# mengcaopku/DCNet

Measured on AMD Instinct MI355X. Metric: clips/sec (T=8, 416x416, bs8) fwd+bwd, higher is better.
Workload: dtype f32; 1 GPU; T=8 416x416 bs8/GPU L=20 fp32, 64 img/GPU/step as pairs, fwd+5 losses+bwd+RMSprop; arith=f16x2-split MFMA, fp32 accumulate, parallelism=dp1, ranks_seen=1, reducer=none, step=hipGraph replay (fwd+losses+bwd+RMSprop), sampler=mt

## Files before the change

dcnet_amd/csrc/coattn.hip:

```cpp
#include "igemm.h"
#include "prof.h"

int tn_gemm_batched(const float* A, int lda, long long a_bs, const float* B, int ldb, long long b_bs,
                    float* C, int ldc, long long c_bs, const float* row_scale,
                    int M, int m_ld, int N, int K, int batch, int accumulate, hipStream_t stream,
                    const unsigned* amax_a = nullptr, const unsigned* amax_b = nullptr);

namespace {

constexpr int EXP_ROWS = 32;

typedef _Float16 f16x4c_t __attribute__((ext_vector_type(4)));
constexpr float E_SPLIT_SCALE = 8192.f;
template <bool SPLIT>
__global__ __launch_bounds__(256) void exp_sums_kernel(float* __restrict__ E, int hw, int ldE, float t,
                                                       float* __restrict__ rsum, float* __restrict__ colpart) {
  __shared__ float red[4][EXP_ROWS];
  const int b = blockIdx.y, rb = blockIdx.x;
  const int i0 = rb * EXP_ROWS;
  float* e = E + ((size_t)b * hw + i0) * ldE;
  float racc[EXP_ROWS];
#pragma unroll
  for (int r = 0; r < EXP_ROWS; ++r) racc[r] = 0.f;
  const int nrow = min(EXP_ROWS, hw - i0);
  for (int j = threadIdx.x * 4; j < ldE; j += 1024) {
    f32x4 v[EXP_ROWS];
#pragma unroll
    for (int r = 0; r < EXP_ROWS; ++r)
      v[r] = r < nrow ? *reinterpret_cast<const f32x4*>(e + (size_t)r * ldE + j) : f32x4{0.f, 0.f, 0.f, 0.f};
    f32x4 cs = {0.f, 0.f, 0.f, 0.f};
#pragma unroll
    for (int r = 0; r < EXP_ROWS; ++r) {
      if (r < nrow) {
        f32x4 o;
#pragma unroll
        for (int k = 0; k < 4; ++k) o[k] = (j + k < hw) ? expf(t * v[r][k] - t) : 0.f;
        if constexpr (SPLIT) {
          const f32x4 ts = o * E_SPLIT_SCALE;
          const f16x4c_t h = {(_Float16)ts[0], (_Float16)ts[1], (_Float16)ts[2], (_Float16)ts[3]};
          const f16x4c_t l = {(_Float16)(ts[0] - (float)h[0]), (_Float16)(ts[1] - (float)h[1]), (_Float16)(ts[2] - (float)h[2]),
                              (_Float16)(ts[3] - (float)h[3])};
          unsigned char* run = reinterpret_cast<unsigned char*>(e + (size_t)r * ldE + (j & ~7)) + (j & 4) * 2;
          *reinterpret_cast<f16x4c_t*>(run) = h;
          *reinterpret_cast<f16x4c_t*>(run + 16) = l;
        } else {
          *reinterpret_cast<f32x4*>(e + (size_t)r * ldE + j) = o;
        }
        cs += o; racc[r] += (o[0] + o[1]) + (o[2] + o[3]);
      }
    }
    *reinterpret_cast<f32x4*>(colpart + ((size_t)rb * gridDim.y + b) * ldE + j) = cs;
  }
  const int lane = threadIdx.x & 63, wave = threadIdx.x >> 6;
#pragma unroll
  for (int r = 0; r < EXP_ROWS; ++r) {
    const float s = wave_sum(racc[r]);
    if (lane == 0) red[wave][r] = s;
  }
  __syncthreads();
  if (threadIdx.x < EXP_ROWS && i0 + threadIdx.x < hw)
    rsum[(size_t)b * hw + i0 + threadIdx.x] = 1.f / (red[0][threadIdx.x] + red[1][threadIdx.x] + red[2][threadIdx.x] + red[3][threadIdx.x]);
}

__global__ __launch_bounds__(256) void colsum_inv_kernel(const float* __restrict__ colpart, int nrb, int b, int hw, int ldE,
                                                         float* __restrict__ cinv) {
  const int j = blockIdx.x * 256 + threadIdx.x, bb = blockIdx.y;
  if (j >= hw) return;
  float s = 0.f;
  for (int rb = 0; rb < nrb; ++rb) s += colpart[((size_t)rb * b + bb) * ldE + j];
  cinv[(size_t)bb * hw + j] = 1.f / s;
}

enum { AM_ONE = 0, AM_DO1, AM_DO2, AM_DO1S, AM_DO2S, AM_DA, AM_DP1, AM_DP2, AM_SLOTS };
__global__ __launch_bounds__(256) void amax_init_kernel(unsigned* __restrict__ w) {
  for (int i = threadIdx.x; i < AM_SLOTS * DCN_AMAX_WORDS; i += 256) w[i] = i < DCN_AMAX_WORDS ? 0x3F800000u : 0u;
}

__global__ __launch_bounds__(256) void rowdot_scale_kernel(const float* __restrict__ d, int ldd, int64_t bsd,
                                                           const float* __restrict__ o, int ldo, int64_t bso, int hw,
                                                           const float* __restrict__ inv, int64_t rows, int c,
                                                           float* __restrict__ delta, float* __restrict__ ds,
                                                           unsigned* __restrict__ amax_d, unsigned* __restrict__ amax_ds) {
  __shared__ float red[4];
  const int lane = threadIdx.x & 63;
  const int64_t row = (int64_t)blockIdx.x * 4 + (threadIdx.x >> 6);
  float vmax = 0.f, s = 0.f;
  if (row < rows) {
    const int64_t bb = row / hw, i = row - bb * hw;
    s = inv[row];
    float acc = 0.f;
    for (int k = lane * 4; k < c; k += 256) {
      const f32x4 dv = *reinterpret_cast<const f32x4*>(d + bb * bsd + i * ldd + k);
      const f32x4 ov = *reinterpret_cast<const f32x4*>(o + bb * bso + i * ldo + k);
      acc += dv[0] * ov[0] + dv[1] * ov[1] + dv[2] * ov[2] + dv[3] * ov[3];
      *reinterpret_cast<f32x4*>(ds + row * c + k) = dv * s;
      vmax = fmaxf(fmaxf(vmax, fmaxf(fabsf(dv[0]), fabsf(dv[1]))), fmaxf(fabsf(dv[2]), fabsf(dv[3])));
    }
    acc = wave_sum(acc);
    if (lane == 0) delta[row] = acc;
  }
  const float vs = wave_max(vmax * s);
  amax_update_block(amax_d, vmax, red);
  __syncthreads();
  amax_update_block(amax_ds, vs, red);
// ... 24 lines not shown
      const f16x4c_t h = *reinterpret_cast<const f16x4c_t*>(run), l = *reinterpret_cast<const f16x4c_t*>(run + 16);
#pragma unroll
      for (int k = 0; k < 4; ++k) e[k] = ((float)h[k] + (float)l[k]) * (1.f / E_SPLIT_SCALE);
    } else {
      e = *reinterpret_cast<const f32x4*>(E + row * ldE + j);
    }
    const f32x4 p1 = *reinterpret_cast<const f32x4*>(dP1 + row * ldE + j);
    const f32x4 p2 = *reinterpret_cast<const f32x4*>(dP2 + row * ldE + j);
    const float ri = rinv[row], di = d1[row];
    f32x4 o;
#pragma unroll
    for (int k = 0; k < 4; ++k) {
      float v = 0.f;
      if (j + k < hw) v = t * e[k] * ((p1[k] - di) * ri + (p2[k] - d2[bb * hw + j + k]) * cinv[bb * hw + j + k]);
      o[k] = v;
    }
    if constexpr (OSPLIT) {
      const f32x4 ts = o * s_out;
      const f16x4c_t h = {(_Float16)ts[0], (_Float16)ts[1], (_Float16)ts[2], (_Float16)ts[3]};
      const f16x4c_t l = {(_Float16)(ts[0] - (float)h[0]), (_Float16)(ts[1] - (float)h[1]), (_Float16)(ts[2] - (float)h[2]),
                          (_Float16)(ts[3] - (float)h[3])};
      unsigned char* run = reinterpret_cast<unsigned char*>(dP1 + row * ldE + (j & ~7)) + (j & 4) * 2;
      *reinterpret_cast<f16x4c_t*>(run) = h;
      *reinterpret_cast<f16x4c_t*>(run + 16) = l;
    } else {
      *reinterpret_cast<f32x4*>(dP1 + row * ldE + j) = o;
      vmax = fmaxf(fmaxf(vmax, fmaxf(fabsf(o[0]), fabsf(o[1]))), fmaxf(fabsf(o[2]), fabsf(o[3])));
    }
  }
  if constexpr (!OSPLIT) amax_update_block(amax_da, vmax, red);
}

__global__ __launch_bounds__(64) void da_bound_kernel(const unsigned* __restrict__ a1, const unsigned* __restrict__ a2, float t,
                                                      unsigned* __restrict__ out) {
  const float b = 2.f * t * (__uint_as_float(amax_read(a1)) + __uint_as_float(amax_read(a2)));
  out[threadIdx.x & (DCN_AMAX_WORDS - 1)] = __float_as_uint(b);
}

inline int ld_pad(int hw) { return (hw + 31) / 32 * 32; }

void gemm_params(IgemmParams& p, const float* A, int lda, long long a_bs, const float* B, int ldb, long long b_bs,
                 float* C, int ldc, long long c_bs, int M, int N, int K, int batch) {
  p = IgemmParams{};
  p.osy = p.osx = p.isy = p.isx = 1; p.dense_out = 1;
  p.in = A; p.ldi = lda; p.in_bs = a_bs; p.wt = B; p.ldw = ldb; p.wt_bs = b_bs; p.out = C; p.ldo = ldc; p.out_bs = c_bs;
  p.ldr = ldc;
  p.N = 1; p.Hi = 1; p.Wi = M; p.Ho = 1; p.Wo = M; p.Hs = 1; p.Ws = M; p.M = M;
  p.Ci = K; p.Co = N; p.ntaps = 1; p.batch = batch;
}

}

static bool on_gemm3(int b, int hw, int c) { return c % 32 == 0 && gemm3_applicable(hw, c, hw, b) && gemm3_applicable(hw, hw, c, b); }

extern "C" int64_t dcn_coattn_fwd_ws(int b, int hw, int c) {
  (void)c;
  return (int64_t)cdiv(hw, EXP_ROWS) * b * ld_pad(hw) + AM_SLOTS * DCN_AMAX_WORDS;
}
extern "C" int64_t dcn_coattn_e_size(int b, int hw) { return (int64_t)b * hw * ld_pad(hw); }
extern "C" int64_t dcn_coattn_saved_size(int b, int hw, int c) {
  return dcn_coattn_e_size(b, hw) + (on_gemm3(b, hw, c) ? (int64_t)2 * b * hw * c : 0);
}

extern "C" int dcn_coattn_fwd(const float* f1, const float* f2, int ldf, int64_t bsf, float* f1_attn, float* f2_attn, int ldo,
                              int64_t bso, float* E, float* rinv, float* cinv, float* ws,
                              int b, int hw, int c, float temperature, void* stream_) {
  hipStream_t stream = (hipStream_t)stream_;
  DCN_CHECK_ARG(f1 && f2 && f1_attn && E && rinv && cinv && ws, "coattn_fwd: null pointer");
  DCN_CHECK_ARG(b > 0 && hw > 0 && c > 0 && c % 32 == 0, "coattn_fwd: bad shape (c=%d must be a multiple of 32)", c);
  if (ldf <= 0) ldf = c;
  if (ldo <= 0) ldo = c;
  DCN_CHECK_ARG(ldf % 4 == 0 && ldo % 4 == 0, "coattn_fwd: ldf/ldo must be multiples of 4");
  if (bsf <= 0) bsf = (int64_t)hw * ldf;
  if (bso <= 0) bso = (int64_t)hw * ldo;
  DCN_CHECK_ARG(bsf % 4 == 0 && bso % 4 == 0, "coattn_fwd: batch strides must be multiples of 4");
  const int ldE = ld_pad(hw);
  unsigned* am = reinterpret_cast<unsigned*>(ws + (int64_t)cdiv(hw, EXP_ROWS) * b * ldE);
  hipLaunchKernelGGL(amax_init_kernel, dim3(1), dim3(256), 0, stream, am);
  DCN_CHECK_LAUNCH("coattn amax_init");
  const unsigned* one = am + AM_ONE * DCN_AMAX_WORDS;
  const int nrb = cdiv(hw, EXP_ROWS);
  const long long bsE = (long long)hw * ldE;
  if (on_gemm3(b, hw, c)) {
    float* f1s = E + dcn_coattn_e_size(b, hw);
    float* f2s = f1s + (int64_t)b * hw * c;
    const long long bss = (long long)hw * c;
    int rc = gemm3_presplit(f1, ldf, bsf, f1s, c, bss, b, hw, c, one, stream);
    if (rc) return rc;
    if ((rc = gemm3_presplit(f2, ldf, bsf, f2s, c, bss, b, hw, c, one, stream))) return rc;
    if ((rc = gemm3_launch(f1s, c, bss, 0, f2s, c, bss, 0, E, ldE, bsE, nullptr, 0, hw, hw, c, b, 0, one, one, stream))) return rc;
    const int pid = prof_begin(12, (double)b * hw * ldE * 8.0, stream);
    hipLaunchKernelGGL(exp_sums_kernel<true>, dim3(nrb, b), dim3(256), 0, stream, E, hw, ldE, temperature, rinv, ws);
    prof_end(pid, stream);
    DCN_CHECK_LAUNCH("exp_sums");
    hipLaunchKernelGGL(colsum_inv_kernel, dim3(cdiv(hw, 256), b), dim3(256), 0, stream, ws, nrb, b, hw, ldE, cinv);
    DCN_CHECK_LAUNCH("colsum_inv");
    if ((rc = gemm3_launch(E, ldE, bsE, 0, f2s, c, bss, 1, f1_attn, ldo, bso, rinv, hw, hw, c, hw, b, 0, one, one, stream))) return rc;
    if (f2_attn) rc = gemm3_launch(E, ldE, bsE, 1, f1s, c, bss, 1, f2_attn, ldo, bso, cinv, hw, hw, c, hw, b, 0, one, one, stream);
    return rc;
  }
  IgemmParams p;
  gemm_params(p, f1, ldf, bsf, f2, ldf, bsf, E, ldE, (long long)hw * ldE, hw, hw, c, b);
  p.amax_a = one; p.amax_b = one;
  int rc = igemm_launch(p, stream);
  if (rc) return rc;
  const int pid = prof_begin(12, (double)b * hw * ldE * 8.0, stream);
  hipLaunchKernelGGL(exp_sums_kernel<false>, dim3(nrb, b), dim3(256), 0, stream, E, hw, ldE, temperature, rinv, ws);
  prof_end(pid, stream);
  DCN_CHECK_LAUNCH("exp_sums");
  hipLaunchKernelGGL(colsum_inv_kernel, dim3(cdiv(hw, 256), b), dim3(256), 0, stream, ws, nrb, b, hw, ldE, cinv);
  DCN_CHECK_LAUNCH("colsum_inv");
  gemm_params(p, E, ldE, (long long)hw * ldE, f2, ldf, bsf, f1_attn, ldo, bso, hw, c, ldE, b);
  p.bmode = 1; p.kvalid = hw; p.row_scale = rinv; p.amax_a = one; p.amax_b = one;
  rc = igemm_launch(p, stream);
  if (rc) return rc;
  if (f2_attn)
    rc = tn_gemm_batched(E, ldE, (long long)hw * ldE, f1, ldf, bsf, f2_attn, ldo, bso,
                         cinv, hw, ldE, c, hw, b, 0, stream, one, one);
  return rc;
}

extern "C" int64_t dcn_coattn_bwd_ws(int b, int hw, int c) {
  return (int64_t)2 * b * hw * ld_pad(hw) + (int64_t)2 * b * hw * c + (int64_t)2 * b * hw + AM_SLOTS * DCN_AMAX_WORDS +
         (on_gemm3(b, hw, c) ? (int64_t)2 * b * hw * c + 4 : 0);
}

extern "C" int dcn_coattn_bwd(const float* f1, const float* f2, int ldf, int64_t bsf,
                              const float* d_f1_attn, const float* d_f2_attn, int lddo, int64_t bsdo,
                              const float* f1_attn, const float* f2_attn, int ldo, int64_t bso,
                              const float* E, const float* rinv, const float* cinv,
                              float* d_f1, float* d_f2, int lddf, int64_t bsdf, int accumulate, float* ws,
                              int b, int hw, int c, float temperature, void* stream_) {
  hipStream_t stream = (hipStream_t)stream_;
  DCN_CHECK_ARG(f1 && f2 && d_f1_attn && d_f2_attn && f1_attn && f2_attn && E && rinv && cinv && d_f1 && d_f2 && ws,
                "coattn_bwd: null pointer");
  DCN_CHECK_ARG(b > 0 && hw > 0 && c > 0 && c % 32 == 0, "coattn_bwd: bad shape");
  if (ldf <= 0) ldf = c;
  if (ldo <= 0) ldo = c;
  if (lddo <= 0) lddo = c;
  if (lddf <= 0) lddf = c;
  if (bsf <= 0) bsf = (int64_t)hw * ldf;
  if (bso <= 0) bso = (int64_t)hw * ldo;
  if (bsdo <= 0) bsdo = (int64_t)hw * lddo;
  if (bsdf <= 0) bsdf = (int64_t)hw * lddf;
  const int ldE = ld_pad(hw);
  const long long rows = (long long)b * hw;
  float* dP1 = ws;
// ... 68 lines not shown
```

dcnet_amd/csrc/gemm3.hip:

```cpp
#include "igemm.h"
#include "prof.h"

namespace {

typedef _Float16 f16x8_t __attribute__((ext_vector_type(8)));
typedef short s16x4 __attribute__((ext_vector_type(4)));
typedef short s16x8 __attribute__((ext_vector_type(8)));
typedef __attribute__((address_space(3))) void lds_void;

#define G3_ABL 0
constexpr unsigned G3_OOB = 0x80000000u;
constexpr int G3_BM = 256, G3_BN = 256, G3_STAGES = 4;
constexpr int G3_TILE = 256 * 64;
constexpr int G3_STAGE = 2 * G3_TILE;
constexpr int G3_LDS = G3_STAGES * G3_STAGE;

__device__ __forceinline__ float g3_pow2_scale(unsigned amax_bits) {
  const int be = (int)((amax_bits >> 23) & 0xFF);
  if (be == 0 || be == 255) return 1.f;
  int e = 14 - (be - 126);
  e = e > 100 ? 100 : (e < -100 ? -100 : e);
  return __uint_as_float((unsigned)(e + 127) << 23);
}

struct G3Params {
  const float* A; const float* B; float* C;
  long long a_bs, b_bs, c_bs;
  int lda, ldb, ldc;
  int M, N, K;
  int a_rows, b_rows;
  int a_cols, b_cols;
  int tiles_m, tiles_n;
  const float* row_scale; long long rs_bs;
  int accumulate;
  const unsigned* amax_a; const unsigned* amax_b;
  unsigned* amax_out;
  int var;
  int abl;
};

__device__ __forceinline__ int g3_tswz(int krow) { return (krow & 1) | ((krow & 2) << 1); }

template <bool AT, bool BT, bool H1 = false>
__global__ __launch_bounds__(512, 1) void gemm3_kernel(const G3Params p) {
  extern __shared__ __attribute__((aligned(1024))) unsigned char smem3g[];
  const int tid = threadIdx.x, lane = tid & 63;
  const int wave = __builtin_amdgcn_readfirstlane(tid >> 6);
  const int wm = wave >> 2, wn = wave & 3;
  const int per_batch = p.tiles_m * p.tiles_n;
  const int lin = xcd_remap(blockIdx.x, gridDim.x);
  const int batch = __builtin_amdgcn_readfirstlane(lin / per_batch), t_ = lin - batch * per_batch;
  const int bm = __builtin_amdgcn_readfirstlane(t_ / p.tiles_n), bn = t_ - bm * p.tiles_n;
  const int m0 = bm * G3_BM, n0 = bn * G3_BN;
  const int kslices = (p.K + 15) >> 4;

  const float* a_base = p.A + batch * p.a_bs + (AT ? 0 : (long long)m0 * p.lda);
  const float* b_base = p.B + batch * p.b_bs + (BT ? 0 : (long long)n0 * p.ldb);
  const int a_rows_left = AT ? p.a_rows : p.a_rows - m0, b_rows_left = BT ? p.b_rows : p.b_rows - n0;
  const long long a_bytes = ((long long)(a_rows_left - 1) * p.lda + p.a_cols) * 4, b_bytes = ((long long)(b_rows_left - 1) * p.ldb + p.b_cols) * 4;
  const __amdgpu_buffer_rsrc_t a_rs = __builtin_amdgcn_make_buffer_rsrc((void*)a_base, 0, a_bytes > 0x7FFFFFF0LL ? 0x7FFFFFF0 : (int)a_bytes, 0x00020000);
  const __amdgpu_buffer_rsrc_t b_rs = __builtin_amdgcn_make_buffer_rsrc((void*)b_base, 0, b_bytes > 0x7FFFFFF0LL ? 0x7FFFFFF0 : (int)b_bytes, 0x00020000);

  unsigned voff[4];
  int sstep_a, sstep_b;
#pragma unroll
  for (int e = 0; e < 2; ++e) {
    const int j = 2 * wave + e;
    if (AT) {
      voff[e] = (unsigned)((long long)j * p.lda * 4 + m0 * 4 + ((lane ^ g3_tswz(j)) << 4));
      if (m0 + ((lane ^ g3_tswz(j)) << 2) >= p.a_cols) voff[e] = G3_OOB;
    } else {
      const int row = 16 * j + (lane >> 2), c = (lane & 3) ^ ((row >> 2) & 3);
      voff[e] = row < a_rows_left ? (unsigned)((long long)row * p.lda * 4 + c * 16) : G3_OOB;
    }
    if (BT) {
      voff[2 + e] = (unsigned)((long long)j * p.ldb * 4 + n0 * 4 + ((lane ^ g3_tswz(j)) << 4));
      if (n0 + ((lane ^ g3_tswz(j)) << 2) >= p.b_cols) voff[2 + e] = G3_OOB;
    } else {
      const int row = 16 * j + (lane >> 2), c = (lane & 3) ^ ((row >> 2) & 3);
      voff[2 + e] = row < b_rows_left ? (unsigned)((long long)row * p.ldb * 4 + c * 16) : G3_OOB;
    }
  }
  sstep_a = AT ? 16 * p.lda * 4 : 64;
  sstep_b = BT ? 16 * p.ldb * 4 : 64;
  const int my_dst = 2 * wave * 1024;

  int k_done = 0;
  auto issue_a = [&]() {
    const bool live = k_done < kslices && !(G3_ABL && (p.abl & 1));
    unsigned char* st = smem3g + (k_done & (G3_STAGES - 1)) * G3_STAGE + my_dst;
    int sa_ = live ? k_done * sstep_a : 0;
    if (G3_ABL && (p.abl & 8)) sa_ = 0;
#pragma unroll
    for (int e = 0; e < 2; ++e)
      __builtin_amdgcn_raw_ptr_buffer_load_lds(a_rs, (lds_void*)(st + e * 1024), 16, (int)(live ? voff[e] : G3_OOB), sa_, 0, 0);
  };
// ... 77 lines not shown
    } else {
#pragma unroll
      for (int ni = 0; ni < 2; ++ni) {
        if (BT) { bh[ni] = tfrag(st, b_rd[ni][0], b_rd[ni][1], 0); if constexpr (!H1) bl[ni] = tfrag(st, b_rd[ni][0], b_rd[ni][1], 1); }
        else { bh[ni] = *reinterpret_cast<const f16x8_t*>(st + b_rd[ni][0]); if constexpr (!H1) bl[ni] = *reinterpret_cast<const f16x8_t*>(st + b_rd[ni][1]); }
      }
#pragma unroll
      for (int mi = 0; mi < 4; ++mi) {
        if (AT) { ah[mi] = tfrag(st, a_rd[mi][0], a_rd[mi][1], 0); if constexpr (!H1) al[mi] = tfrag(st, a_rd[mi][0], a_rd[mi][1], 1); }
        else { ah[mi] = *reinterpret_cast<const f16x8_t*>(st + a_rd[mi][0]); if constexpr (!H1) al[mi] = *reinterpret_cast<const f16x8_t*>(st + a_rd[mi][1]); }
      }
    }
    if (p.var >= 1) {
      issue_a();
      if (wm == 1) asm volatile("s_waitcnt vmcnt(%0)" :: "n"((G3_STAGES - 2) * 4 - 2) : "memory");
    } else {
      issue();
      if (wm == 1) asm volatile("s_waitcnt vmcnt(%0)" :: "n"((G3_STAGES - 2) * 4) : "memory");
    }
    asm volatile("s_waitcnt lgkmcnt(0)" ::: "memory");
    __builtin_amdgcn_s_barrier();
    asm volatile("" ::: "memory");
    if (G3_ABL && (p.abl & 4)) {
#pragma unroll
      for (int mi = 0; mi < 4; ++mi) { asm volatile("" :: "v"(ah[mi]), "v"(al[mi])); }
#pragma unroll
      for (int ni = 0; ni < 2; ++ni) { asm volatile("" :: "v"(bh[ni]), "v"(bl[ni])); }
    } else {
      __builtin_amdgcn_s_setprio(1);
      if constexpr (!H1) {
#pragma unroll
        for (int mi = 0; mi < 4; ++mi)
#pragma unroll
          for (int ni = 0; ni < 2; ++ni) acc[mi][ni] = __builtin_amdgcn_mfma_f32_32x32x16_f16(al[mi], bh[ni], acc[mi][ni], 0, 0, 0);
        if (p.var == 2) issue_b();
#pragma unroll
        for (int mi = 0; mi < 4; ++mi)
#pragma unroll
          for (int ni = 0; ni < 2; ++ni) acc[mi][ni] = __builtin_amdgcn_mfma_f32_32x32x16_f16(ah[mi], bl[ni], acc[mi][ni], 0, 0, 0);
      } else if (p.var == 2) issue_b();
#pragma unroll
      for (int mi = 0; mi < 4; ++mi)
#pragma unroll
        for (int ni = 0; ni < 2; ++ni) acc[mi][ni] = __builtin_amdgcn_mfma_f32_32x32x16_f16(ah[mi], bh[ni], acc[mi][ni], 0, 0, 0);
      __builtin_amdgcn_s_setprio(0);
    }
    if (p.var == 1) issue_b();
    if (wm == 0) asm volatile("s_waitcnt vmcnt(%0)" :: "n"((G3_STAGES - 2) * 4) : "memory");
  }
  if (wm == 0) __builtin_amdgcn_s_barrier();
  asm volatile("s_waitcnt vmcnt(0)" ::: "memory");

  const float dq = 1.f / (g3_pow2_scale(amax_read(p.amax_a)) * g3_pow2_scale(amax_read(p.amax_b)));
  float* __restrict__ cb = p.C + batch * p.c_bs;
  const float* rs = p.row_scale ? p.row_scale + batch * p.rs_bs : nullptr;
  float vmax = 0.f;
#pragma unroll
  for (int mi = 0; mi < 4; ++mi)
#pragma unroll
    for (int r = 0; r < 16; ++r) {
      const int m = m0 + wm * 128 + mi * 32 + 4 * g + (r & 3) + 8 * (r >> 2);
      if (m >= p.M) continue;
      const float f = rs ? dq * rs[m] : dq;
#pragma unroll
      for (int ni = 0; ni < 2; ++ni) {
        const int n = n0 + wn * 64 + ni * 32 + (lane & 31);
        if (n >= p.N) continue;
        float v = acc[mi][ni][r] * f;
        float* dst = cb + (long long)m * p.ldc + n;
        if (p.accumulate) v += *dst;
        *dst = v;
        vmax = fmaxf(vmax, fabsf(v));
      }
    }
  if (p.amax_out) {
    vmax = wave_max(vmax);
    if (lane == 0) amax_update(p.amax_out, vmax, blockIdx.x * 8 + wave);
  }
}

__global__ __launch_bounds__(256) void presplit_kernel(const float* __restrict__ src, int ld, long long bs, float* __restrict__ dst, int ldd,
                                                        long long bsd, int rows, int c, long long total8, const unsigned* __restrict__ amax) {
  const float s = g3_pow2_scale(amax_read(amax));
  const int c8 = c >> 3;
  for (long long i = (long long)blockIdx.x * 256 + threadIdx.x; i < total8; i += (long long)gridDim.x * 256) {
    const long long row_all = i / c8; const int o = (int)(i - row_all * c8);
    const long long b = row_all / rows; const int row = (int)(row_all - b * rows);
    const float* sp = src + b * bs + (long long)row * ld + o * 8;
    const f32x4 x0 = *reinterpret_cast<const f32x4*>(sp) * s, x1 = *reinterpret_cast<const f32x4*>(sp + 4) * s;
    f16x8_t h, l;
#pragma unroll
    for (int e = 0; e < 4; ++e) { h[e] = (_Float16)x0[e]; h[4 + e] = (_Float16)x1[e]; }
#pragma unroll
    for (int e = 0; e < 4; ++e) { l[e] = (_Float16)(x0[e] - (float)h[e]); l[4 + e] = (_Float16)(x1[e] - (float)h[4 + e]); }
    float* dp = dst + b * bsd + (long long)row * ldd + o * 8;
    *reinterpret_cast<f16x8_t*>(dp) = h;
    *reinterpret_cast<f16x8_t*>(dp + 4) = l;
  }
}

int g_gemm3 = 1;

int g_gemm3_h1 = 1;

template <bool AT, bool BT, bool H1>
int launch3g_(const G3Params& p, int grid, hipStream_t stream) {
  static DcnPerDeviceFlag attr_once;
  if (attr_once.first()) {
    (void)hipFuncSetAttribute(reinterpret_cast<const void*>(&gemm3_kernel<AT, BT, H1>), hipFuncAttributeMaxDynamicSharedMemorySize, G3_LDS);
  }
  hipLaunchKernelGGL((gemm3_kernel<AT, BT, H1>), dim3(grid), dim3(512), G3_LDS, stream, p);
  return DCN_OK;
}
template <bool AT, bool BT>
int launch3g(const G3Params& p, int grid, hipStream_t stream) {
  if (g_gemm3_h1 && igemm_precision() == 2) return launch3g_<AT, BT, true>(p, grid, stream);
  return launch3g_<AT, BT, false>(p, grid, stream);
}

}

void gemm3_set_tuning(int v) { g_gemm3 = v; }
void gemm3_set_h1(int v) { g_gemm3_h1 = v; }

bool gemm3_applicable(int M, int N, int K, int batch) {
  return g_gemm3 && (igemm_precision() == 4 || igemm_precision() == 2) && M >= 512 && N >= 256 && K >= 64 && batch >= 1;
}

int gemm3_presplit(const float* src, int ld, long long bs, float* dst, int ldd, long long bsd, int batch, int rows, int c,
                   const unsigned* amax, hipStream_t stream) {
  DCN_CHECK_ARG(src && dst && amax && c % 8 == 0 && ld % 4 == 0 && ldd % 4 == 0 && bs % 4 == 0 && bsd % 4 == 0, "gemm3_presplit: bad argument");
  const long long total8 = (long long)batch * rows * (c / 8);
  long long g = (total8 + 255) / 256; if (g > 16384) g = 16384;
  hipLaunchKernelGGL(presplit_kernel, dim3((int)g), dim3(256), 0, stream, src, ld, bs, dst, ldd, bsd, rows, c, total8, amax);
  DCN_CHECK_LAUNCH("gemm3_presplit");
  return DCN_OK;
}

int gemm3_launch(const float* A, int lda, long long a_bs, int at, const float* B, int ldb, long long b_bs, int bt,
                 float* C, int ldc, long long c_bs, const float* row_scale, long long rs_bs,
                 int M, int N, int K, int batch, int accumulate, const unsigned* amax_a, const unsigned* amax_b, hipStream_t stream,
                 unsigned* amax_out) {
  DCN_CHECK_ARG(A && B && C && amax_a && amax_b, "gemm3: null pointer");
  DCN_CHECK_ARG(lda % 4 == 0 && ldb % 4 == 0 && a_bs % 4 == 0 && b_bs % 4 == 0 && (((uintptr_t)A | (uintptr_t)B) & 15) == 0, "gemm3: 16-byte rows");
  G3Params p{};
  p.A = A; p.B = B; p.C = C; p.a_bs = a_bs; p.b_bs = b_bs; p.c_bs = c_bs; p.lda = lda; p.ldb = ldb; p.ldc = ldc;
  p.M = M; p.N = N; p.K = K;
  const int k16 = (K + 15) / 16 * 16;
  p.a_rows = at ? K : M; p.b_rows = bt ? K : N;
  p.a_cols = at ? (M + 7) / 8 * 8 : k16; p.b_cols = bt ? (N + 7) / 8 * 8 : k16;
  DCN_CHECK_ARG(p.a_cols <= lda && p.b_cols <= ldb, "gemm3: rows shorter than the tile reads (lda=%d ldb=%d)", lda, ldb);
  p.tiles_m = cdiv(M, G3_BM); p.tiles_n = cdiv(N, G3_BN);
  p.row_scale = row_scale; p.rs_bs = rs_bs; p.accumulate = accumulate; p.amax_a = amax_a; p.amax_b = amax_b; p.amax_out = amax_out; p.abl = (g_gemm3 >> 4) & 15; p.var = g_gemm3 >> 8;
  const int grid = p.tiles_m * p.tiles_n * batch;
  const int pid = prof_begin(40, 2.0 * batch * (double)M * N * K, stream);
  int rc;
  if (at) rc = bt ? launch3g<true, true>(p, grid, stream) : DCN_ERR_ARG;
  else rc = bt ? launch3g<false, true>(p, grid, stream) : launch3g<false, false>(p, grid, stream);
  prof_end(pid, stream);
  DCN_CHECK_ARG(rc == DCN_OK, "gemm3: no A^T . B^T form");
  DCN_CHECK_LAUNCH("gemm3");
  return DCN_OK;
}

extern "C" int dcn_gemm3_supported(int m, int n, int k, int batch) { return gemm3_applicable(m, n, k, batch) ? 1 : 0; }

extern "C" int dcn_gemm3_presplit(const float* src, int ld, int64_t bs, float* dst, int ldd, int64_t bsd, int batch, int rows, int c,
                                  const uint32_t* amax, void* stream) {
  return gemm3_presplit(src, ld, bs, dst, ldd, bsd, batch, rows, c, amax, (hipStream_t)stream);
}

extern "C" int dcn_gemm3(const float* a, int lda, int64_t a_bs, int a_t, const float* b, int ldb, int64_t b_bs, int b_t,
                         float* c, int ldc, int64_t c_bs, const float* row_scale, int64_t rs_bs,
                         int m, int n, int k, int batch, int accumulate, const uint32_t* amax_a, const uint32_t* amax_b, void* stream) {
  DCN_CHECK_ARG(m > 0 && n > 0 && k > 0 && batch > 0, "gemm3: empty problem");
  return gemm3_launch(a, lda, a_bs, a_t, b, ldb, b_bs, b_t, c, ldc, c_bs, row_scale, rs_bs, m, n, k, batch, accumulate, amax_a, amax_b,
                      (hipStream_t)stream, nullptr);
}
```

dcnet_amd/csrc/igemm.h:

```cpp
#pragma once
#include "common.h"

#define IGEMM_MAX_TAPS 16


struct IgemmParams {
  const float* in;
  const float* wt;
  const float* f8;
  const unsigned* amax_a;
  const unsigned* amax_b;
  const void* wt16;
  const float* b_scale;
  unsigned* amax_out;
  float* out;
  const float* scale;
  const float* shift;
  const float* residual;
  float* stats;
  const float* row_scale;
  int batch;
  long long in_bs, wt_bs, out_bs;
  int bmode;
  int kvalid;
// ... 14 lines not shown
  const float* bt_y; const float* bt_mean; const float* bt_invstd; const float* bt_gamma; const float* bt_beta;
  int bt_act; float bt_slope;
  const unsigned char* a_scale8; const unsigned char* b_scale8;
};
inline double epilogue_reads(const IgemmParams& p) { return 1.0 + (p.accumulate ? 1.0 : 0.0) + (p.residual ? 1.0 : 0.0) + (p.bt_y ? 1.0 : 0.0); }
bool igemm_tap_capable(const IgemmParams& p);

int igemm_grid_m(int M, int Co, int ntaps);
int igemm_launch(const IgemmParams& p, hipStream_t stream);
bool igemm_will_presplit(long long rows, int Co, int ntaps, int Ci);

bool conv3_applicable(const IgemmParams& p, int precision, int gran);
int conv3_launch(const IgemmParams& p, int gran, hipStream_t stream);
void conv3_set_tuning(int key, int value);
bool conv3x_takes(const IgemmParams& p, int gran);
int conv3x_launch(const IgemmParams& p, int gran, hipStream_t stream);
void conv3x_set_tuning(int v);
int conv3b_bm(int M, int Co, int Wi);
bool conv3b_takes(const IgemmParams& p);
int conv3b_launch(const IgemmParams& p, int out_f32, hipStream_t stream);
void conv3b_set_tuning(int v);

bool conv1_applicable(const IgemmParams& p, int precision, int gran);
int conv1_launch(const IgemmParams& p, int gran, hipStream_t stream);
void conv1_set_tuning(int key, int value);
int conv1b_grid_m(int M, int Co, int ntaps, int s1_w = 0);
int conv1b_launch(const IgemmParams& p, int out_f32, hipStream_t stream);
int conv1q_grid_m(int M, int Co);
int conv1q_launch(const IgemmParams& p, int out_f32, hipStream_t stream);
bool conv2b_takes(int M, int Co, int ntaps);
int conv2b_launch(const IgemmParams& p, int out_f32, hipStream_t stream);
void conv2b_set_tuning(int v);


bool stem_applicable(const IgemmParams& p, const float* scratch);
int stem_launch(const IgemmParams& p, float* scratch, hipStream_t stream);
void stem_set_tuning(int v);

bool dgrad2_applicable(int n, int h, int wd, int cin, int cout, int ksize, int stride, int accumulate);
struct DcnBnTap { const float* y; const float* mean; const float* invstd; const float* gamma; const float* beta; int act; float slope;
                  float* stats; int stats_rows; };
int nconv1_launch_b16(int mode, const void* x, int ldi, const void* w16, void* y, int ldo, float* stats, int stats_rows,
                      int n, int h, int wd, int stride, hipStream_t stream);
int dgrad2_launch_b16(const void* dy, int lddy, const void* wt16, void* dx, int n, int h, int wd, int cin, int accumulate, hipStream_t stream);
int dgrad2_grid(int n, int h, int wd, int cin);
int dgrad2_launch(const float* dy, int lddy, const float* wt, float* dx, int n, int h, int wd, int cin, int accumulate,
                  const uint32_t* amax_dy, const uint32_t* amax_w, const DcnBnTap* tap, hipStream_t stream);
void nconv_set_tuning(int v);
void gemm3_set_tuning(int v);
void gemm3_set_h1(int v);
bool gemm3_applicable(int M, int N, int K, int batch);
int gemm3_presplit(const float* src, int ld, long long bs, float* dst, int ldd, long long bsd, int batch, int rows, int c,
                   const unsigned* amax, hipStream_t stream);
int gemm3_launch(const float* A, int lda, long long a_bs, int at, const float* B, int ldb, long long b_bs, int bt,
                 float* C, int ldc, long long c_bs, const float* row_scale, long long rs_bs,
                 int M, int N, int K, int batch, int accumulate, const unsigned* amax_a, const unsigned* amax_b, hipStream_t stream,
                 unsigned* amax_out = nullptr);
int igemm_precision();
struct DcnPreAct { const float* scale; const float* shift; int act; float slope; };
bool nconv1_applicable(int mode, int n, int h, int wd, int cin, int cout, int ksize, int stride);
int nconv1_launch(int mode, const float* x, int ldi, const float* w, float* y, int ldo, float* stats, int stats_rows,
                  int n, int h, int wd, int stride, const uint32_t* amax_x, const uint32_t* amax_w, const DcnPreAct* pre, hipStream_t stream);
```

dcnet_amd/csrc/igemm.hip:

```cpp
#include "igemm.h"
#include "prof.h"
#include <type_traits>

namespace {


typedef unsigned int u32x4 __attribute__((ext_vector_type(4)));
typedef __bf16 bf16x8 __attribute__((ext_vector_type(8)));
constexpr unsigned OOB = 0x80000000u;

__device__ __forceinline__ f32x4 buf_load16(__amdgpu_buffer_rsrc_t r, unsigned voff, unsigned soff) {
  return __builtin_bit_cast(f32x4, __builtin_amdgcn_raw_buffer_load_b128(r, voff, soff, 0));
}
__device__ __forceinline__ __amdgpu_buffer_rsrc_t make_rsrc(const float* base, long long bytes) {
  const unsigned n = bytes > 0x7FFFFFF0LL ? 0x7FFFFFF0u : (unsigned)bytes;
  return __builtin_amdgcn_make_buffer_rsrc((void*)base, 0, n, 0x00020000);
}

typedef short s16x4 __attribute__((ext_vector_type(4)));
typedef short s16x8 __attribute__((ext_vector_type(8)));
__device__ __forceinline__ float pow2_scale(unsigned amax_bits) {
  const int be = (int)((amax_bits >> 23) & 0xFF);
  if (be == 0 || be == 255) return 1.f;
  int e = 14 - (be - 126);
// ... 565 lines not shown
int g_tile64 = 1;

inline int tile_bm(int M, int Co, int ntaps, int Ci) {
  if (Co <= 32) return 256;
  if (Co <= 64) return (g_tile64 && g_precision >= 1 && !g_force_bm && ntaps >= 2 && ntaps * Ci >= 256) ? 256 : 128;
  if (g_force_bm) return g_force_bm;
  (void)M;
  return 128;
}

}

int igemm_grid_m(int M, int Co, int ntaps) { return cdiv(M, tile_bm(M, Co, ntaps, 32)); }

void wgrad_set_split(int v);
void wgrad_set_lds_pad(int kb);
void wgrad_set_abl(int v);
void wgrad_set_target(int v);
void wgrad_set_wide64(int v);
void wgrad_set_target_small(int v);
void wgrad_set_w3_b16(int v);
void wgrad_set_w9_b16(int v);
void wgrad_set_target_b16(int v, int small);
void wgrad3_set_tuning(int key, int value);
void wgrad_set_w1x(int v);
void bn_set_pc(int v);
void conv_set_merge(int v);
void conv_set_d2_b16(int v);
void conv_set_n1_b16(int v);
void score_set_tuning(int key, int value);
void bn_set_tuning(int v);
void wgrad9_set_tuning(int key, int value);
void wgrad_set_slab_fold(int v);

extern "C" int dcn_set_tuning(const char* key, int value) {
  const char k = key ? key[0] : 0;
  if (k == 'S' && key[1] == 'l') { wgrad_set_slab_fold(value); return DCN_OK; }
  if (k == '2') { conv2b_set_tuning(value); return DCN_OK; }
  if (k == 'H') { gemm3_set_h1(value); return DCN_OK; }
  if (k == 'q' && key[1] == 't') { wgrad_set_target_b16(value, 0); return DCN_OK; }
  if (k == 'q' && key[1] == 's') { wgrad_set_target_b16(value, 1); return DCN_OK; }
  if (k == 'w' && key[1] == '3') { wgrad_set_w3_b16(value); return DCN_OK; }
  if (k == 'b' && key[1] == 'w') { conv1_set_tuning(4, value); return DCN_OK; }
  if (k == 'b' && key[1] == 't') { conv1_set_tuning(5, value); return DCN_OK; }
  if (k == '1') { conv1_set_tuning(key[1] == 's' ? 1 : (key[1] == 'f' ? 2 : (key[1] == 'w' ? 3 : (key[1] == 't' ? 6 : 0))), value); return DCN_OK; }
  if (k == '3') { if (key[1] == 'h') { conv3b_set_tuning(value); return DCN_OK; }
    if (key[1] == 'd') { conv3x_set_tuning(value); return DCN_OK; }
    conv3_set_tuning(key[1] == 'b' ? 1 : key[1] == 'a' ? 2 : key[1] == 'l' ? 3 : key[1] == 'm' ? 4 : 0, value); return DCN_OK; }
  if (k == 'N' && key[1] == 'b') { conv_set_n1_b16(value); return DCN_OK; }
  if (k == 'D') { conv_set_d2_b16(value); return DCN_OK; }
  if (k == '9' && key[1] == 'b') { wgrad_set_w9_b16(value); return DCN_OK; }
  if (k == '9') { wgrad9_set_tuning(key[1] == 't' && key[2] == 'a' && key[3] == 'r' ? 1 : 0, value); return DCN_OK; }
  if (k == 'G') { gemm3_set_tuning(value); return DCN_OK; }
  if (k == 'N') { nconv_set_tuning(value); return DCN_OK; }
  if (k == 'd') { bn_set_tuning(value); return DCN_OK; }
  if (k == 'e') { score_set_tuning(0, value); return DCN_OK; }
  if (k == 'f') { score_set_tuning(1, value); return DCN_OK; }
  if (k == 'l') { wgrad_set_lds_pad(value); return DCN_OK; }
  if (k == 'j') { stem_set_tuning(value); return DCN_OK; }
  if (k == 'm') { conv_set_merge(value); return DCN_OK; }
  if (k == 'Y') { wgrad_set_w1x(value); return DCN_OK; }
  if (k == 'U') { wgrad3_set_tuning(2, value); return DCN_OK; }
  if (k == 'u') { wgrad3_set_tuning(0, value); return DCN_OK; }
  if (k == 'v') { wgrad3_set_tuning(1, value); return DCN_OK; }
  if (k == 'B') { bn_set_pc(value); return DCN_OK; }
  if (k == 'z') { wgrad_set_target_small(value); return DCN_OK; }
  if (k == 'c') { wgrad_set_wide64(value); return DCN_OK; }
  if (k == 'x') { wgrad_set_target(value); return DCN_OK; }
  if (k == 'w') { wgrad_set_split(value); return DCN_OK; }
  if (k == 'p') { g_precision = value; wgrad_set_split(value == 3 ? 2 : value); return DCN_OK; }
  if (k == 'b') g_force_bm = value;
  else if (k == 'k') g_force_bk = value;
  else if (k == 'n') g_nn_split = value;
  else if (k == 'o') g_occ3 = value;
  else if (k == 'h') g_h2_occ3 = value;
  else if (k == 'g') g_h2_k32 = value;
  else if (k == 'r') g_h2_narrow = value;
  else if (k == 'q') g_h2_bk = value;
  else if (k == 'y') g_h2_presplit = value;
  else if (k == 't') g_tile64 = value;
  else if (k == 'a') { g_abl = value; wgrad_set_abl(value); }
  else if (k == 's') g_split = value;
  else { dcn_set_error("set_tuning: unknown key"); return DCN_ERR_ARG; }
  return DCN_OK;
}

int igemm_precision() { return g_precision; }

bool igemm_will_presplit(long long rows, int Co, int ntaps, int Ci) {
  if (g_precision != 4 || !g_h2_presplit || g_split || rows < 1024 || Co <= 32) return false;
  if (Co <= 64) return tile_bm((int)rows, Co, ntaps, Ci) == 256;
  return tile_bm((int)rows, Co, ntaps, Ci) == 128;
}

bool igemm_tap_capable(const IgemmParams& p) {
  if (!p.stats || p.ncls || p.batch > 1 || !p.dense_out) return false;
  const int gran = tile_bm(p.M, p.Co, p.ntaps, 32);
  return conv3_applicable(p, g_precision, gran) || conv1_applicable(p, g_precision, gran);
}

int igemm_launch(const IgemmParams& p, hipStream_t stream) {
  DCN_CHECK_ARG(p.in && p.wt && p.out, "igemm: null pointer");
  DCN_CHECK_ARG(p.M > 0 && p.Co > 0 && p.Ci > 0, "igemm: empty problem (M=%d Co=%d Ci=%d)", p.M, p.Co, p.Ci);
  DCN_CHECK_ARG(p.c4 ? (p.Ci == 4) : (p.Ci % 32 == 0), "igemm: Ci=%d must be a multiple of 32 (or 4 in c4 mode)", p.Ci);
  DCN_CHECK_ARG(p.ntaps >= 1 && p.ntaps <= IGEMM_MAX_TAPS, "igemm: ntaps=%d", p.ntaps);
  DCN_CHECK_ARG(p.ldi % 4 == 0 && p.ldw % 4 == 0, "igemm: ldi=%d ldw=%d must be multiples of 4 floats", p.ldi, p.ldw);
// ... 36 lines not shown
```

Before: 87.77 clips/s.

## Fuse coattention exp, f16 split store and row/column sums into GEMM epilogue

Adds an EXP epilogue to the gemm3 NT kernel. It applies exp(t*s - t) to the accumulators, writes E directly in the hi/lo f16 split layout, and emits per-4-column row partial sums and per-32-row column partials. A small gsum_rinv kernel then reduces the row partials into rinv, which replaces the separate exp_sums pass that re-read and re-wrote the full E matrix. The cost is extra DPP shuffles and scattered stores in the GEMM epilogue, one more template instantiation, and extra workspace for the row partials.

```diff
diff --git a/dcnet_amd/csrc/coattn.hip b/dcnet_amd/csrc/coattn.hip
--- a/dcnet_amd/csrc/coattn.hip
+++ b/dcnet_amd/csrc/coattn.hip
@@ -50,6 +50,34 @@
       }
     }
     *reinterpret_cast<f32x4*>(colpart + ((size_t)rb * gridDim.y + b) * ldE + j) = cs;
+  }
+  const int lane = threadIdx.x & 63, wave = threadIdx.x >> 6;
+#pragma unroll
+  for (int r = 0; r < EXP_ROWS; ++r) {
+    const float s = wave_sum(racc[r]);
+    if (lane == 0) red[wave][r] = s;
+  }
+  __syncthreads();
+  if (threadIdx.x < EXP_ROWS && i0 + threadIdx.x < hw)
+    rsum[(size_t)b * hw + i0 + threadIdx.x] = 1.f / (red[0][threadIdx.x] + red[1][threadIdx.x] + red[2][threadIdx.x] + red[3][threadIdx.x]);
+}
+
+__global__ __launch_bounds__(256) void gsum_rinv_kernel(const float* __restrict__ gsum, int hw, int ldE, float* __restrict__ rsum) {
+  __shared__ float red[4][EXP_ROWS];
+  const int b = blockIdx.y, rb = blockIdx.x;
+  const int i0 = rb * EXP_ROWS, l4 = ldE >> 2;
+  const float* gp = gsum + ((size_t)b * hw + i0) * l4;
+  float racc[EXP_ROWS];
+#pragma unroll
+  for (int r = 0; r < EXP_ROWS; ++r) racc[r] = 0.f;
+  const int nrow = min(EXP_ROWS, hw - i0);
+  for (int q = threadIdx.x; q < l4; q += 256) {
+    float v[EXP_ROWS];
+#pragma unroll
+    for (int r = 0; r < EXP_ROWS; ++r) v[r] = r < nrow ? gp[(size_t)r * l4 + q] : 0.f;
+#pragma unroll
+    for (int r = 0; r < EXP_ROWS; ++r)
+      if (r < nrow) racc[r] += v[r];
   }
   const int lane = threadIdx.x & 63, wave = threadIdx.x >> 6;
 #pragma unroll
@@ -180,10 +208,12 @@
 }
 
 static bool on_gemm3(int b, int hw, int c) { return c % 32 == 0 && gemm3_applicable(hw, c, hw, b) && gemm3_applicable(hw, hw, c, b); }
+static int g_coattn_fuse = 1;
+void coattn_set_fuse(int v) { g_coattn_fuse = v; }
+static bool fused(int b, int hw, int c) { return g_coattn_fuse && on_gemm3(b, hw, c); }
 
 extern "C" int64_t dcn_coattn_fwd_ws(int b, int hw, int c) {
-  (void)c;
-  return (int64_t)cdiv(hw, EXP_ROWS) * b * ld_pad(hw) + AM_SLOTS * DCN_AMAX_WORDS;
+  return (int64_t)cdiv(hw, EXP_ROWS) * b * ld_pad(hw) + AM_SLOTS * DCN_AMAX_WORDS + (fused(b, hw, c) ? (int64_t)b * hw * (ld_pad(hw) / 4) : 0);
 }
 extern "C" int64_t dcn_coattn_e_size(int b, int hw) { return (int64_t)b * hw * ld_pad(hw); }
 extern "C" int64_t dcn_coattn_saved_size(int b, int hw, int c) {
@@ -216,11 +246,19 @@
     int rc = gemm3_presplit(f1, ldf, bsf, f1s, c, bss, b, hw, c, one, stream);
     if (rc) return rc;
     if ((rc = gemm3_presplit(f2, ldf, bsf, f2s, c, bss, b, hw, c, one, stream))) return rc;
-    if ((rc = gemm3_launch(f1s, c, bss, 0, f2s, c, bss, 0, E, ldE, bsE, nullptr, 0, hw, hw, c, b, 0, one, one, stream))) return rc;
-    const int pid = prof_begin(12, (double)b * hw * ldE * 8.0, stream);
-    hipLaunchKernelGGL(exp_sums_kernel<true>, dim3(nrb, b), dim3(256), 0, stream, E, hw, ldE, temperature, rinv, ws);
-    prof_end(pid, stream);
-    DCN_CHECK_LAUNCH("exp_sums");
+    if (fused(b, hw, c)) {
+      G3Epi ep{};
+      ep.mode = G3_EPI_EXP; ep.t = temperature; ep.n_pad = ldE; ep.colpart = ws; ep.gsum = reinterpret_cast<float*>(am + AM_SLOTS * DCN_AMAX_WORDS);
+      if ((rc = gemm3_launch(f1s, c, bss, 0, f2s, c, bss, 0, E, ldE, bsE, nullptr, 0, hw, hw, c, b, 0, one, one, stream, nullptr, &ep))) return rc;
+      hipLaunchKernelGGL(gsum_rinv_kernel, dim3(nrb, b), dim3(256), 0, stream, ep.gsum, hw, ldE, rinv);
+      DCN_CHECK_LAUNCH("gsum_rinv");
+    } else {
+      if ((rc = gemm3_launch(f1s, c, bss, 0, f2s, c, bss, 0, E, ldE, bsE, nullptr, 0, hw, hw, c, b, 0, one, one, stream))) return rc;
+      const int pid = prof_begin(12, (double)b * hw * ldE * 8.0, stream);
+      hipLaunchKernelGGL(exp_sums_kernel<true>, dim3(nrb, b), dim3(256), 0, stream, E, hw, ldE, temperature, rinv, ws);
+      prof_end(pid, stream);
+      DCN_CHECK_LAUNCH("exp_sums");
+    }
     hipLaunchKernelGGL(colsum_inv_kernel, dim3(cdiv(hw, 256), b), dim3(256), 0, stream, ws, nrb, b, hw, ldE, cinv);
     DCN_CHECK_LAUNCH("colsum_inv");
     if ((rc = gemm3_launch(E, ldE, bsE, 0, f2s, c, bss, 1, f1_attn, ldo, bso, rinv, hw, hw, c, hw, b, 0, one, one, stream))) return rc;
diff --git a/dcnet_amd/csrc/gemm3.hip b/dcnet_amd/csrc/gemm3.hip
--- a/dcnet_amd/csrc/gemm3.hip
+++ b/dcnet_amd/csrc/gemm3.hip
@@ -37,11 +37,24 @@
   unsigned* amax_out;
   int var;
   int abl;
+  int nbatch;
+  G3Epi epi;
 };
 
+constexpr float G3_E_SCALE = 8192.f;
+
+__device__ __forceinline__ void g3_store_split(float* row, int n, float ts, bool odd) {
+  const _Float16 h = (_Float16)ts, l = (_Float16)(ts - (float)h);
+  const unsigned hb = __builtin_bit_cast(unsigned short, h), lb = __builtin_bit_cast(unsigned short, l);
+  const unsigned got = (unsigned)__builtin_amdgcn_mov_dpp((int)(odd ? hb : lb), 0xB1, 0xF, 0xF, false);
+  unsigned char* run = reinterpret_cast<unsigned char*>(row + (n & ~7)) + 2 * (n & 7);
+  if (odd) *reinterpret_cast<unsigned*>(run + 14) = got | (lb << 16);
+  else *reinterpret_cast<unsigned*>(run) = hb | (got << 16);
+}
+
 __device__ __forceinline__ int g3_tswz(int krow) { return (krow & 1) | ((krow & 2) << 1); }
 
-template <bool AT, bool BT, bool H1 = false>
+template <bool AT, bool BT, bool H1 = false, int EPI = G3_EPI_PLAIN>
 __global__ __launch_bounds__(512, 1) void gemm3_kernel(const G3Params p) {
   extern __shared__ __attribute__((aligned(1024))) unsigned char smem3g[];
   const int tid = threadIdx.x, lane = tid & 63;
@@ -225,6 +238,57 @@
   asm volatile("s_waitcnt vmcnt(0)" ::: "memory");
 
   const float dq = 1.f / (g3_pow2_scale(amax_read(p.amax_a)) * g3_pow2_scale(amax_read(p.amax_b)));
+  if constexpr (EPI == G3_EPI_EXP) {
+    const float t = p.epi.t;
+    const bool odd = lane & 1;
+    float* ce = p.C + batch * p.c_bs;
+#pragma unroll
+    for (int mi = 0; mi < 4; ++mi)
+#pragma unroll
+      for (int r = 0; r < 16; ++r) {
+        const int m = m0 + wm * 128 + mi * 32 + 4 * g + (r & 3) + 8 * (r >> 2);
+#pragma unroll
+        for (int ni = 0; ni < 2; ++ni) {
+          const int n = n0 + wn * 64 + ni * 32 + (lane & 31);
+          acc[mi][ni][r] = (m < p.M && n < p.N) ? expf(t * (acc[mi][ni][r] * dq) - t) : 0.f;
+        }
+        float* row = ce + (long long)m * p.ldc;
+        float* grow = p.epi.gsum + ((long long)batch * p.M + m) * (p.ldc >> 2);
+#pragma unroll
+        for (int ni = 0; ni < 2; ++ni) {
+          const int n = n0 + wn * 64 + ni * 32 + (lane & 31);
+          const float e = acc[mi][ni][r];
+          const float e01 = e + __int_as_float(__builtin_amdgcn_mov_dpp(__float_as_int(e), 0xB1, 0xF, 0xF, false));
+          const float e0123 = e01 + __int_as_float(__builtin_amdgcn_mov_dpp(__float_as_int(e01), 0x4E, 0xF, 0xF, false));
+          const float g4 = __int_as_float(__builtin_amdgcn_mov_dpp(__float_as_int(e0123), 0x104, 0xF, 0xF, false));
+          const float g8 = __int_as_float(__builtin_amdgcn_mov_dpp(__float_as_int(e0123), 0x108, 0xF, 0xF, false));
+          const float g12 = __int_as_float(__builtin_amdgcn_mov_dpp(__float_as_int(e0123), 0x10C, 0xF, 0xF, false));
+          if (m < p.M && n < p.epi.n_pad) {
+            g3_store_split(row, n, e * G3_E_SCALE, odd);
+            if ((lane & 15) == 0) *reinterpret_cast<f32x4*>(grow + (n >> 2)) = f32x4{e0123, g4, g8, g12};
+          }
+        }
+      }
+#pragma unroll
+    for (int mi = 0; mi < 4; ++mi) {
+      const int mb = m0 + wm * 128 + mi * 32;
+#pragma unroll
+      for (int ni = 0; ni < 2; ++ni) {
+        float s = 0.f;
+#pragma unroll
+        for (int q = 0; q < 8; ++q) {
+          float x = s;
+#pragma unroll
+          for (int i = 0; i < 4; ++i) x = x + acc[mi][ni][4 * (q >> 1) + i];
+          const float other = __shfl_xor(x, 32);
+          s = g == (q & 1) ? x : other;
+        }
+        const int n = n0 + wn * 64 + ni * 32 + (lane & 31);
+        if (g == 0 && mb < p.M && n < p.N) p.epi.colpart[((long long)(mb >> 5) * p.nbatch + batch) * p.ldc + n] = s;
+      }
+    }
+    return;
+  }
   float* __restrict__ cb = p.C + batch * p.c_bs;
   const float* rs = p.row_scale ? p.row_scale + batch * p.rs_bs : nullptr;
   float vmax = 0.f;
@@ -276,19 +340,19 @@
 
 int g_gemm3_h1 = 1;
 
-template <bool AT, bool BT, bool H1>
+template <bool AT, bool BT, bool H1, int EPI>
 int launch3g_(const G3Params& p, int grid, hipStream_t stream) {
   static DcnPerDeviceFlag attr_once;
   if (attr_once.first()) {
-    (void)hipFuncSetAttribute(reinterpret_cast<const void*>(&gemm3_kernel<AT, BT, H1>), hipFuncAttributeMaxDynamicSharedMemorySize, G3_LDS);
-  }
-  hipLaunchKernelGGL((gemm3_kernel<AT, BT, H1>), dim3(grid), dim3(512), G3_LDS, stream, p);
+    (void)hipFuncSetAttribute(reinterpret_cast<const void*>(&gemm3_kernel<AT, BT, H1, EPI>), hipFuncAttributeMaxDynamicSharedMemorySize, G3_LDS);
+  }
+  hipLaunchKernelGGL((gemm3_kernel<AT, BT, H1, EPI>), dim3(grid), dim3(512), G3_LDS, stream, p);
   return DCN_OK;
 }
-template <bool AT, bool BT>
+template <bool AT, bool BT, int EPI = G3_EPI_PLAIN>
 int launch3g(const G3Params& p, int grid, hipStream_t stream) {
-  if (g_gemm3_h1 && igemm_precision() == 2) return launch3g_<AT, BT, true>(p, grid, stream);
-  return launch3g_<AT, BT, false>(p, grid, stream);
+  if (g_gemm3_h1 && igemm_precision() == 2) return launch3g_<AT, BT, true, EPI>(p, grid, stream);
+  return launch3g_<AT, BT, false, EPI>(p, grid, stream);
 }
 
 }
@@ -313,9 +377,14 @@
 int gemm3_launch(const float* A, int lda, long long a_bs, int at, const float* B, int ldb, long long b_bs, int bt,
                  float* C, int ldc, long long c_bs, const float* row_scale, long long rs_bs,
                  int M, int N, int K, int batch, int accumulate, const unsigned* amax_a, const unsigned* amax_b, hipStream_t stream,
-                 unsigned* amax_out) {
+                 unsigned* amax_out, const G3Epi* epi) {
   DCN_CHECK_ARG(A && B && C && amax_a && amax_b, "gemm3: null pointer");
-  DCN_CHECK_ARG(lda % 4 == 0 && ldb % 4 == 0 && a_bs % 4 == 0 && b_bs % 4 == 0 && (((uintptr_t)A | (uintptr_t)B) & 15) == 0, "gemm3: 16-byte rows");
+  if (epi && epi->mode != G3_EPI_PLAIN) {
+    DCN_CHECK_ARG(epi->mode == G3_EPI_EXP && epi->colpart && epi->gsum && !at && !bt && !accumulate && !row_scale && !amax_out &&
+                  epi->n_pad >= N && epi->n_pad <= ldc && epi->n_pad % 32 == 0 && ldc % 32 == 0 && c_bs % 8 == 0 && (((uintptr_t)C) & 15) == 0 &&
+                  (((uintptr_t)epi->gsum) & 15) == 0,
+                  "gemm3: fused epilogue on an NT product with 8-column runs only");
+  }
   G3Params p{};
   p.A = A; p.B = B; p.C = C; p.a_bs = a_bs; p.b_bs = b_bs; p.c_bs = c_bs; p.lda = lda; p.ldb = ldb; p.ldc = ldc;
   p.M = M; p.N = N; p.K = K;
@@ -325,11 +394,15 @@
   DCN_CHECK_ARG(p.a_cols <= lda && p.b_cols <= ldb, "gemm3: rows shorter than the tile reads (lda=%d ldb=%d)", lda, ldb);
   p.tiles_m = cdiv(M, G3_BM); p.tiles_n = cdiv(N, G3_BN);
   p.row_scale = row_scale; p.rs_bs = rs_bs; p.accumulate = accumulate; p.amax_a = amax_a; p.amax_b = amax_b; p.amax_out = amax_out; p.abl = (g_gemm3 >> 4) & 15; p.var = g_gemm3 >> 8;
+  p.nbatch = batch;
+  if (epi) p.epi = *epi;
   const int grid = p.tiles_m * p.tiles_n * batch;
   const int pid = prof_begin(40, 2.0 * batch * (double)M * N * K, stream);
   int rc;
   if (at) rc = bt ? launch3g<true, true>(p, grid, stream) : DCN_ERR_ARG;
-  else rc = bt ? launch3g<false, true>(p, grid, stream) : launch3g<false, false>(p, grid, stream);
+  else if (bt) rc = launch3g<false, true>(p, grid, stream);
+  else if (p.epi.mode == G3_EPI_EXP) rc = launch3g<false, false, G3_EPI_EXP>(p, grid, stream);
+  else rc = launch3g<false, false>(p, grid, stream);
   prof_end(pid, stream);
   DCN_CHECK_ARG(rc == DCN_OK, "gemm3: no A^T . B^T form");
   DCN_CHECK_LAUNCH("gemm3");
diff --git a/dcnet_amd/csrc/igemm.h b/dcnet_amd/csrc/igemm.h
--- a/dcnet_amd/csrc/igemm.h
+++ b/dcnet_amd/csrc/igemm.h
@@ -90,10 +90,13 @@
 bool gemm3_applicable(int M, int N, int K, int batch);
 int gemm3_presplit(const float* src, int ld, long long bs, float* dst, int ldd, long long bsd, int batch, int rows, int c,
                    const unsigned* amax, hipStream_t stream);
+enum { G3_EPI_PLAIN = 0, G3_EPI_EXP = 1 };
+struct G3Epi { int mode; float t; int n_pad; float* colpart; float* gsum; };
 int gemm3_launch(const float* A, int lda, long long a_bs, int at, const float* B, int ldb, long long b_bs, int bt,
                  float* C, int ldc, long long c_bs, const float* row_scale, long long rs_bs,
                  int M, int N, int K, int batch, int accumulate, const unsigned* amax_a, const unsigned* amax_b, hipStream_t stream,
-                 unsigned* amax_out = nullptr);
+                 unsigned* amax_out = nullptr, const G3Epi* epi = nullptr);
+void coattn_set_fuse(int v);
 int igemm_precision();
 struct DcnPreAct { const float* scale; const float* shift; int act; float slope; };
 bool nconv1_applicable(int mode, int n, int h, int wd, int cin, int cout, int ksize, int stride);
diff --git a/dcnet_amd/csrc/igemm.hip b/dcnet_amd/csrc/igemm.hip
--- a/dcnet_amd/csrc/igemm.hip
+++ b/dcnet_amd/csrc/igemm.hip
@@ -641,6 +641,7 @@
   if (k == '9' && key[1] == 'b') { wgrad_set_w9_b16(value); return DCN_OK; }
   if (k == '9') { wgrad9_set_tuning(key[1] == 't' && key[2] == 'a' && key[3] == 'r' ? 1 : 0, value); return DCN_OK; }
   if (k == 'G') { gemm3_set_tuning(value); return DCN_OK; }
+  if (k == 'C') { coattn_set_fuse(value); return DCN_OK; }
   if (k == 'N') { nconv_set_tuning(value); return DCN_OK; }
   if (k == 'd') { bn_set_tuning(value); return DCN_OK; }
   if (k == 'e') { score_set_tuning(0, value); return DCN_OK; }
```

Result: no change. 87.82 clips/s, median of 6 (+0.1%).
